# SaeedRahmani/MPC-RL_for_AVs

Measured on AMD Instinct MI355X. Metric: MPC solves/sec (horizon=20, batch=4096), higher is better.
Workload: dtype f64

## Files before the change

### __graft_entry__.py

```python
from __future__ import annotations

import os
import subprocess
import sys

ROOT = os.path.dirname(os.path.abspath(__file__))
if ROOT not in sys.path:
    sys.path.insert(0, ROOT)
ORACLE = os.path.join(ROOT, "oracle")


def abi_version_of_header() -> int:
    import re
    with open(os.path.join(ROOT, "include", "mpc_mi355x.h")) as f:
        m = re.search(r"^#define\s+MPC_ABI_VERSION\s+(\d+)", f.read(), re.M)
    if not m:
        raise RuntimeError("MPC_ABI_VERSION not found in include/mpc_mi355x.h")
    return int(m.group(1))


def build() -> None:
    from mpc_rl_for_avs_amd import _build, engine
    path = _build.build(force=_build.is_stale())
    print(f"[build] {path}")
    subprocess.run(["make", "-C", ORACLE, "-s"], check=True)
    print(f"[build] {os.path.join(ORACLE, '_build', 'libmpc_oracle.so')}")
    wave_ops_suite = os.path.exists(os.path.join(ROOT, "tests", "wave_ops_cases.py"))
    for lib, src in (("libcpu_wave.so", "cpu_wave_harness.cpp"), ("libcpu_wave_spare.so", "cpu_wave_spare_harness.cpp"),
                     ("libcpu_ltv.so", "cpu_ltv_harness.cpp"),
                     ("libcpu_preamble.so", "cpu_preamble_harness.cpp"), ("libcpu_synth_env.so", "cpu_synth_env_harness.cpp"),
                     ("libcpu_traffic_env.so", "cpu_traffic_env_harness.cpp"),
                     ("libcpu_rollout_glue.so", "cpu_rollout_glue_harness.cpp"), ("libcpu_sde_glue.so", "cpu_sde_glue_harness.cpp"),
                     ("libcpu_wave_ops.so", "cpu_wave_ops_harness.cpp")):
        if lib == "libcpu_wave_ops.so" and not wave_ops_suite:
            continue
        harness = os.path.join(ROOT, "tests", "_build", lib)
        os.makedirs(os.path.dirname(harness), exist_ok=True)
        subprocess.run(["g++", "-O2", "-fPIC", "-shared", "-std=c++17", "-Wno-unknown-pragmas", "-ffp-contract=off",
                        "-o", harness, os.path.join(ROOT, "tests", src)], check=True)
        print(f"[build] {harness}")
    if wave_ops_suite:
        probe = os.path.join(ROOT, "tests", "_build", "libdev_wave_ops.so")
        subprocess.run([_build._hipcc(), "--offload-arch=gfx950", "-O3", "-std=c++17", "-shared", "-fPIC", "-o", probe,
                        os.path.join(ROOT, "tests", "dev_wave_ops.hip")], check=True)
        print(f"[build] {probe}")
    lib = engine.load_library()
    want = abi_version_of_header()
    got = lib.mpc_version()
    assert got == want, f"libmpc_mi355x.so reports ABI {got}, include/mpc_mi355x.h declares {want}: stale library?"
    import mpc_rl_for_avs_amd.pure_mpc
    import mpc_rl_for_avs_amd.pure_mpc_linear


def smoke() -> None:
    if ORACLE not in sys.path:
        sys.path.insert(0, ORACLE)
    import numpy as np
    from mpc_rl_for_avs_amd import engine, synth
    from mpc_rl_for_avs_amd.reference_path import reference_states
    import oracle_lib

    inp = synth.solver_inputs(64, 4, seed=11)
    eng = engine.MPCEngine(horizon=20, max_iter=100, device=0)
    got = eng.solve_batch(inp["state"], inp["ego_index"], inp["weights"], inp["is_collide"], vref=inp["vref"],
                          others=inp["others"], collision_cost=True)
    want = oracle_lib.solve_batch(reference_states(), inp["state"], inp["ego_index"], inp["weights"],
                                  inp["is_collide"], vref=inp["vref"], others=inp["others"], collision_cost=True,
                                  max_iter=100, xy_bounds=False)
    conv = lambda st: (st == 0) | ((st >= 5) & (st <= 7))
    both = conv(got["status"]) & conv(want["status"])
    assert both.sum() >= 60, f"too few converged instances: gpu {got['status']}, oracle {want['status']}"
    assert np.array_equal(got["status"], want["status"]), "status mismatch"
    err = np.abs(got["u0"] - want["u0"]).max(axis=1) / np.maximum(1.0, np.abs(want["u0"]).max(axis=1))
    assert err[both].max() < 1e-4, f"u0 mismatch {err[both].max():.3e}"
    print(f"[smoke] {both.sum()}/64 converged on both, max rel |u0_gpu - u0_oracle| = {err[both].max():.2e}")
    import kkt_batch
    import nlp_batch
    sel = np.nonzero(conv(got["status"]))[0]
    p = nlp_batch.Batch.build(reference_states(), inp["state"], inp["ego_index"], inp["weights"], inp["is_collide"],
                              vref=inp["vref"], others=inp["others"], collision_cost=True).take(sel)
    cert = kkt_batch.certify(p, got["X"][sel], got["U"][sel], eps_c=1e-8 / kkt_batch.objective_scale(p))
    assert cert["stationarity"].max() <= 1e-8 and cert["feasibility"].max() <= 1e-10, cert
# ... 20 lines not shown
```

### mpc-rl_for_avs_amd/csrc/mpc_engine.hip

```cpp
#include <hip/hip_runtime.h>

#include <atomic>
#include <cassert>
#include <chrono>
#include <cmath>
#include <cstdio>
#include <cstring>
#include <new>
#include <string>
#include <vector>

#include "../../include/mpc_mi355x.h"
#include "mpc_core.hpp"
#include "mpc_ltv.hpp"
#include "mpc_wave.hpp"
#include "mpc_wave_dev.hpp"
#include "mpc_preamble.hpp"
#include "mpc_preamble_wave.hpp"
#include "mpc_synth_lanes.hpp"
#include "mpc_rollout_glue.hpp"
#include "mpc_drive_metrics.hpp"
#include "mpc_perception.hpp"
#include "mpc_interaction.hpp"
#include "mpc_episode_stats.hpp"

namespace {

thread_local std::string g_last_error;

int fail(int code, const std::string &msg) {
    g_last_error = msg;
    return code;
}

#define HIP_TRY(expr)                                                                              \
    do {                                                                                           \
        hipError_t e_ = (expr);                                                                    \
        if (e_ != hipSuccess)                                                                      \
            return fail(MPC_ERR_HIP, std::string(#expr) + ": " + hipGetErrorString(e_));          \
    } while (0)

constexpr int kBlock = 64;
constexpr int kMaxDevices = 64;
constexpr int kWaveOcc = 3, kWaveOccGeneric = 3;
constexpr int kWaveOccGenericCC = 2;
constexpr int kWaveOccLat = 2, kLatDepth = 4;
constexpr int kRelaxLat = 7;
constexpr bool wave_spare_lds(int NC, int OCC, int RELAX) { return NC > 0 && OCC == kWaveOccLat && RELAX == kRelaxLat; }

template <int NC, int RELAX = 0, bool SPARE = false>
struct WaveCtx : mpc::wave::WaveOpsT<RELAX> {
    static constexpr int kN = NC;
    static constexpr bool kSpareLds = SPARE;
    const double *table;
    int e0, M;
    __device__ __forceinline__ WaveCtx(mpc::wave::lds_double_t *l, const double *t, int e, int m)
        : mpc::wave::WaveOpsT<RELAX>{l}, table(t), e0(mpc::ego_row0(e, m)), M(m) {}
    __device__ __forceinline__ void tick(int) const {}
    __device__ __forceinline__ double ref(int k, int c) const {
        int idx = e0 + k;
        idx = idx > M - 1 ? M - 1 : idx;
        idx = idx < 0 ? 0 : idx;
        return table[idx * mpc::REF_COLS + c];
    }
    __device__ __forceinline__ double refv(int k) const {
        int idx = e0 + k;
        idx = idx > M - 1 ? M - 1 : idx;
        idx = idx < 0 ? 0 : idx;
        return table[M * mpc::REF_COLS + idx];
    }
};

template <bool CC, class CTX>
__device__ __forceinline__ void stage_problem(CTX &ctx, const mpc::SolveParams &P, int b, int lane, int N, int SL,
                                              const double *__restrict__ ref5, int M, const double *__restrict__ vref,
                                              const double *__restrict__ others, int Vin) {
    const int OTH = SL * (N + 1) + mpc::wave::SC_SIZE;
    for (int node = lane; node <= N; node += kBlock) {
        double rv;
        if (vref) {
            rv = vref[(size_t)b * (N + 1) + node];
        } else {
            int idx = ctx.e0 + node;
            idx = idx > M - 1 ? M - 1 : idx;
            idx = idx < 0 ? 0 : idx;
            rv = ref5[M * mpc::REF_COLS + idx];
        }
        ctx.st(node * SL + mpc::wave::W_RV, rv);
    }
    if (CC && lane < P.V) {
        const double *ov = others + ((size_t)b * Vin + lane) * 4;
        const double sp = ov[2] * P.dt, hh = ov[3];
        ctx.st(OTH + lane * 4 + 0, ov[0]);
        ctx.st(OTH + lane * 4 + 1, ov[1]);
        ctx.st(OTH + lane * 4 + 2, sp * cos(hh));
        ctx.st(OTH + lane * 4 + 3, sp * sin(hh));
    }
}

template <bool CC, int NC, int OCC, int RELAX>
__global__ __launch_bounds__(kBlock, OCC) void mpc_solve_wave_kernel(
    mpc::SolveParams P, int B, const double *__restrict__ ref5, int M, const double *__restrict__ state,
    const int32_t *__restrict__ ego_index, const double *__restrict__ vref, const double *__restrict__ weights,
    const uint8_t *__restrict__ is_collide, const double *__restrict__ others, int Vin,
    const int32_t *__restrict__ nveh, double w_collision, const double *u_init, int u_shift, uint8_t *u_valid,
    double *__restrict__ u0_out, double *U_out, double *__restrict__ X_out, int32_t *__restrict__ status_out,
    int32_t *__restrict__ iters_out, const int32_t *__restrict__ order) {
    extern __shared__ double smem[];
    const int N = NC > 0 ? NC : P.N;
    if ((int)blockIdx.x >= B) return;
    const int b = order ? order[blockIdx.x] : (int)blockIdx.x;
    if (nveh) P.V = min(P.V, max(0, nveh[b]));
    const int lane = threadIdx.x;
    constexpr int SL = mpc::wave::stage_slots(CC);
    using Ctx = WaveCtx<NC, RELAX, wave_spare_lds(NC, OCC, RELAX)>;
    Ctx ctx((mpc::wave::lds_double_t *)smem, ref5, ego_index[b], M);
    stage_problem<CC>(ctx, P, b, lane, N, SL, ref5, M, vref, others, Vin);
    __syncthreads();
    double x0[4];
#pragma unroll
    for (int i = 0; i < 4; ++i) x0[i] = state[(size_t)b * 4 + i];
    const bool collide = is_collide[b] != 0;
    const double ws_ = collide ? 100.0 : weights[(size_t)b * 3 + 0];
    const double wcoll = (CC && collide) ? 3000.0 * w_collision : 0.0;
    mpc::wave::Solver<CC, Ctx> solver(P, ctx, x0, ws_, weights[(size_t)b * 3 + 1], weights[(size_t)b * 3 + 2], wcoll);
    int status, iters, cur;
    double kkt;
    const bool warm = u_init != nullptr && (u_valid == nullptr || u_valid[b] != 0);
    if (warm && lane < N) {
        const int src = min(lane + u_shift, N - 1);
        ctx.st(lane * SL + mpc::wave::W_U + 0, mpc::warm_clamp(u_init[((size_t)b * N + src) * 2 + 0], 0));
        ctx.st(lane * SL + mpc::wave::W_U + 1, mpc::warm_clamp(u_init[((size_t)b * N + src) * 2 + 1], 1));
    }
    __syncthreads();
    solver.solve(status, iters, cur, kkt, warm);
    __syncthreads();
    const int CB = cur * 6;
    if (P.strict_kink && (status == MPC_STATUS_CONVERGED_ON_KINK || status == MPC_STATUS_ACCEPTABLE_ON_KINK))
        status = MPC_STATUS_KINK_UNSOLVED;
    if (lane == 0 && u_valid && U_out) u_valid[b] = MPC_STATUS_IS_SOLVED(status) ? 1 : 0;
    if (lane < 2) u0_out[(size_t)b * 2 + lane] = ctx.ld(CB + mpc::wave::W_U + lane);
    if (U_out && lane < N) {
        U_out[((size_t)b * N + lane) * 2 + 0] = ctx.ld(lane * SL + CB + mpc::wave::W_U + 0);
        U_out[((size_t)b * N + lane) * 2 + 1] = ctx.ld(lane * SL + CB + mpc::wave::W_U + 1);
    }
    if (X_out)
        for (int node = lane; node <= N; node += kBlock)
#pragma unroll
            for (int i = 0; i < 4; ++i)
                X_out[((size_t)b * (N + 1) + node) * 4 + i] = ctx.ld(node * SL + CB + mpc::wave::W_X + i);
    if (lane == 0) {
        if (status_out) status_out[b] = status;
        if (iters_out) iters_out[b] = iters;
    }
}

__global__ __launch_bounds__(64) void mpc_timer_kernel(long long ticks) {
    const long long t0 = wall_clock64();
    while (wall_clock64() - t0 < ticks) __builtin_amdgcn_s_sleep(8);
}

constexpr double kOrderStanding = 0.1, kOrderNear = 15.0, kOrderTurn = 0.05;
constexpr int kOrderBehind = 5;
__device__ __forceinline__ int order_tier(const uint8_t *is_collide, const double *state, const double *others, int V,
                                          const int32_t *nveh, const int32_t *ego, const double *ref5, int M, int N, int i) {
    const double *x = state + (size_t)i * 4;
    if (x[3] < kOrderStanding) return 0;
    if (is_collide[i] != 0) {
// ... 1681 lines not shown
```

### mpc-rl_for_avs_amd/csrc/mpc_wave.hpp

```cpp
#pragma once

#include "mpc_core.hpp"

namespace mpc {
namespace wave {

constexpr int kLanes = 64;
constexpr int kTrials = 4;
constexpr double kProjKeep = 0.1;
constexpr double kProjKeepEnd = 1e-3, kProjEndMu = 1e-6;
constexpr int kGnWatch = 4, kGnSkip = 4;
constexpr double kGnEndMu = 1e-2;
constexpr int kDwProbe = 4;
constexpr int kBoostIter = 28;
constexpr double kOpenLoopStep = 1e-9;
constexpr double kAcceptableTol = 1e-6;
constexpr int kAcceptableIter = 15;
constexpr double kRegMax = 1.0;
constexpr double kKappaEps = 30.0;
constexpr double kMinSlack = 1e-14;
constexpr double kInitPush = 1e-2;

enum : int {
    W_X = 0,
// ... 6 lines not shown
    W_Y = 32,
    W_KX = 36,
    W_KP = 44,
    W_KF = 48,
    W_RV = 50,
    W_ONE = 51,
    W_DTC = 52,
    W_SLOTS = 53,
    W_LX = 53,
    W_Q = 55,
    W_QG = 58,
    W_ZW = 61,
    W_WJ = 62,
    W_CROSS = 63,
    W_SLOTS_CC = 65
};
constexpr int kZeroWord = W_LIN + 2;
enum : int { LIN_A02 = 0, LIN_A12 = 1, LIN_A03 = 4, LIN_A13 = 5, LIN_A23 = 6, LIN_B01 = 8, LIN_B11 = 9, LIN_B21 = 10 };
enum : int { W_DXY = W_LX, W_GW = W_Q, W_DZW = W_Q + 1 };
static_assert(kTrials == 4, "the trial areas below are laid out for four trials");
MPC_HD constexpr int trial_x(bool, int t, int TB) { return t == 0 ? TB : (t == 1 ? W_LIN : (t == 2 ? W_LIN + 6 : W_KX)); }
MPC_HD constexpr int trial_u(bool cc, int t, int TB) { return trial_x(cc, t, TB); }
enum : int {
    SC_SPARE = 0,
    SC_TRIG = 4,
    SC_LOG = SC_TRIG + kTrigWords,
    SC_BND = SC_LOG + kLogWords,
    SC_K = SC_BND + 8,
    SC_NB = SC_K + 6,
    SC_SIZE = SC_NB + 3
};
enum : int { K_SF = 0, K_RD, K_RC, K_QTT, K_Q33, K_MUMIN };
constexpr int kMaxHorizon = kLanes;
enum : int {
    A_L00 = W_KX + 0, A_L01 = W_KX + 1, A_L11 = W_KX + 2, A_H22 = W_KX + 3, A_H23 = W_KX + 4, A_H33 = W_KX + 5,
    A_WTD = W_KX + 6, A_WVD = W_KX + 7, A_H66 = W_KP + 0, A_H77 = W_KP + 1, A_HV6 = W_KP + 2, A_HV7 = W_KF + 0,
    A_HV4 = W_KF + 1,
    A_HV0 = W_X,
    A_HV5 = W_U
};

constexpr int kPreSlots = 12;
enum : int { PQ = 0, PB = 8 };
constexpr double kNoBound = 1e300;

MPC_HD constexpr int stage_slots(bool cc) { return (cc ? W_SLOTS_CC : W_SLOTS) + kPreSlots; }

MPC_HD constexpr int spare_doubles(bool cc, int N, int V) { return cc ? 2 * V * (N + 1) : 0; }
template <class CTX, class = void>
struct spare_lds { static constexpr bool value = false; };
template <class CTX>
struct spare_lds<CTX, decltype((void)CTX::kSpareLds)> { static constexpr bool value = CTX::kSpareLds; };

MPC_HD constexpr int lds_doubles(bool cc, int N, int V, bool spare = false) {
    return stage_slots(cc) * (N + 1) + SC_SIZE + (cc ? 4 * V : 0) + (spare ? spare_doubles(cc, N, V) : 0);
}

enum : int {
    T_PREP = 0, T_ADJOINT, T_DUALRES, T_RIC_INIT, T_RIC_SCALARS, T_RIC_L1, T_RIC_L2, T_RIC_2X2, T_RIC_L4, T_LINEAR,
    T_RATIOS, T_ROLL_DYN, T_ROLL_COST, T_DUALUPD,
    T_R_FEEDBACK, T_R_CLAMP, T_R_DYN, T_R_STORE, T_R_CHECK, T_R_PROJ, T_R_LDSW, T_COUNT
};
template <class CTX, class = void>
struct fine_ticks { static constexpr bool value = false; };
template <class CTX>
struct fine_ticks<CTX, decltype((void)CTX::kFine)> { static constexpr bool value = CTX::kFine; };

template <class T>
struct PerLane {
#if defined(__HIPCC__)
    T v;
    MPC_HD T &at(int) { return v; }
#else
    T v[kLanes];
    MPC_HD T &at(int lane) { return v[lane]; }
#endif
};

MPC_HD bool ratio_greater(double n2, double d2, double n1, double d1) {
    const double a = n2 * d1, b = n1 * d2;
    return a > b || (a == b && d2 > d1);
}

#if !defined(__HIPCC__)
inline int row_partner(int l, int step) {
    return step == 0 ? (l ^ 1) : (step == 1 ? (l ^ 2) : (step == 2 ? ((l & ~7) | (7 - (l & 7))) : ((l & ~15) | (15 - (l & 15)))));
}
template <class T, class OP>
inline void host_row_reduce(PerLane<T> &p, OP op) {
    for (int step = 0; step < 4; ++step) {
        T nv[kLanes];
        for (int l = 0; l < kLanes; ++l) nv[l] = op(p.v[l], p.v[row_partner(l, step)]);
        for (int l = 0; l < kLanes; ++l) p.v[l] = nv[l];
    }
}
template <class T, class OP>
inline T host_reduce(PerLane<T> &p, OP op) {
    host_row_reduce(p, op);
    return op(op(p.v[0], p.v[16]), op(p.v[32], p.v[48]));
}
#endif

MPC_HD constexpr int stage_transition_word(int r, int c, int lin, int zero, int one, int dtw) {
    const int key = 8 * r + c;
    int w = zero;
    w = (r < 4 && r == c) ? one : w;
// ... 22 lines not shown
    double x0[4];
    double ws_, wc_, wd_, wcoll;
    double sf = 1.0;
    MPC_HD double SF() const { return sc(SC_K + K_SF); }
    MPC_HD double RD() const { return sc(SC_K + K_RD); }
    MPC_HD double RC() const { return sc(SC_K + K_RC); }
    MPC_HD double WS() const { return c.fresh(ws_); }
    MPC_HD double WC() const { return c.fresh(wc_); }
    MPC_HD double WD() const { return c.fresh(wd_); }
    MPC_HD double WCOLL() const { return c.fresh(wcoll); }

    MPC_HD Solver(const SolveParams &P_, CTX &c_, const double *x0_, double ws, double wc, double wd, double wcl)
        : P(P_), c(c_), N(CTX::kN > 0 ? CTX::kN : P_.N), SL(stage_slots(CC)), SCR(SL * (N + 1)), OTH(SCR + SC_SIZE),
          SPP(OTH + (CC ? 4 * P_.V : 0)), dt(P_.dt), ws_(c_.uni(ws)), wc_(c_.uni(wc)), wd_(c_.uni(wd)), wcoll(c_.uni(wcl)) {
        x0[0] = x0_[0]; x0[1] = x0_[1]; x0[2] = x0_[2]; x0[3] = x0_[3];
    }
    MPC_HD double S(int k, int slot) const { return c.ld(k * SL + slot); }
    MPC_HD void S(int k, int slot, double v) { c.st(k * SL + slot, v); }
    MPC_HD double sc(int i) const { return c.ld(SCR + i); }
    MPC_HD void sc(int i, double v) { c.st(SCR + i, v); }
    MPC_HD double oth(int j, int q) const { return c.ld(OTH + j * 4 + q); }
    MPC_HD double veh_x(int j, int k) const { return kSpare ? c.ld(SPP + 2 * (j * (N + 1) + k)) : oth(j, 0) + k * oth(j, 2); }
    MPC_HD double veh_y(int j, int k) const { return kSpare ? c.ld(SPP + 2 * (j * (N + 1) + k) + 1) : oth(j, 1) + k * oth(j, 3); }
    MPC_HD void init_spare() {
        if (!kSpare || !CC) return;
        c.phase([&](int lane) {
            for (int k = lane; k <= N; k += kLanes)
                for (int j = 0; j < P.V; ++j) {
                    c.st(SPP + 2 * (j * (N + 1) + k), oth(j, 0) + k * oth(j, 2));
                    c.st(SPP + 2 * (j * (N + 1) + k) + 1, oth(j, 1) + k * oth(j, 3));
                }
        });
    }
    MPC_HD double xlo(int i) const { return sc(SC_BND + 0 + 2 * i); }
    MPC_HD double xhi(int i) const { return sc(SC_BND + 1 + 2 * i); }
    MPC_HD double ulo(int i) const { return sc(SC_BND + 4 + 2 * i); }
    MPC_HD double uhi(int i) const { return sc(SC_BND + 5 + 2 * i); }
    MPC_HD double flog(double x) const {
        double K[kLogWords];
        for (int i = 0; i < kLogWords; ++i) K[i] = sc(SC_LOG + i);
        return log_pos(K, x);
    }
    MPC_HD TrigCoef trig() const {
        TrigCoef K;
        for (int i = 0; i < 6; ++i) {
            K.s[i] = sc(SC_TRIG + i);
            K.c[i] = sc(SC_TRIG + 6 + i);
        }
        return K;
    }

    PerLane<double> red_a, red_b, red_c, red_w;
    PerLane<int> ls_feas;
    int any_wall = 0;
    MPC_HD int f_word(int r, int c) const {
        const int w = stage_transition_word(r, c, 0, 1000, 1001, 1002);
        int t = w;
        t = w == 1000 ? kZeroWord : t;
        t = w == 1001 ? W_ONE : t;
        t = w == 1002 ? W_DTC : t;
        t = w == 0 ? W_LIN + LIN_A02 : t;
        t = w == 1 ? W_LIN + LIN_A03 : t;
        t = w == 2 ? W_LIN + LIN_A12 : t;
        t = w == 3 ? W_LIN + LIN_A13 : t;
        t = w == 4 ? W_LIN + LIN_A23 : t;
        t = w == 5 ? W_LIN + LIN_B01 : t;
        t = w == 6 ? W_LIN + LIN_B11 : t;
        t = w == 7 ? W_LIN + LIN_B21 : t;
        return t;
    }
    PerLane<int> r_a, r_b, r_lxx, r_lux, r_m, r_lx, r_lu, r_kx;
    MPC_HD void set_roles4(int AB) {
        c.lanes([&](int lane_) {
            const int lane = c.opaque(lane_);
            const int hi = lane >> 4, blk = (lane >> 2) & 3, lo = lane & 3;
            const int zero = kZeroWord;
            r_a.at(lane_) = f_word(hi, lo);
            r_b.at(lane_) = f_word(hi, lo < 2 ? 6 + lo : 4);
            const int a = hi < lo ? hi : lo, b = hi < lo ? lo : hi;
            const int key = a * 4 + b;
            int slot = zero;
            slot = key == 0 * 4 + 0 ? A_L00 : slot;
            slot = key == 0 * 4 + 1 ? A_L01 : slot;
            slot = key == 1 * 4 + 1 ? A_L11 : slot;
            slot = key == 2 * 4 + 2 ? A_H22 : slot;
            slot = key == 2 * 4 + 3 ? A_H23 : slot;
            slot = key == 3 * 4 + 3 ? A_H33 : slot;
            r_lxx.at(lane_) = slot;
            r_lux.at(lane_) = hi == 1 ? (lo == 2 ? A_WTD : (lo == 3 ? A_WVD : zero)) : zero;
            r_m.at(lane_) = (hi == 0 && lo == 0) ? A_H66 : ((hi == 1 && lo == 1) ? A_H77 : zero);
            r_lx.at(lane_) = lo == 0 ? AB + A_HV0 + hi : zero;
            r_lu.at(lane_) = lo == 0 ? (hi == 0 ? A_HV6 : (hi == 1 ? A_HV7 : zero)) : zero;
            int out = -1;
            out = (blk == 0 && hi < 2) ? W_KX + 2 * lo + hi : out;
            out = (blk == 1 && hi < 2 && lo < 2) ? W_KP + 2 * lo + hi : out;
            out = (blk == 2 && hi < 2 && lo == 0) ? W_KF + hi : out;
            r_kx.at(lane_) = out;
        });
    }

    MPC_HD void load_stage4(int k, int AB, PerLane<double> &RA, PerLane<double> &RB, PerLane<double> &QXX, PerLane<double> &QUX,
                            PerLane<double> &M, PerLane<double> &QX, PerLane<double> &QU, double &lp0, double &lp1) {
        c.lanes([&](int lane) {
            const int base = k * SL;
            auto word = [&](int w) { return c.ld(base + w); };
            RA.at(lane) = word(r_a.at(lane));
            RB.at(lane) = word(r_b.at(lane));
            QXX.at(lane) = word(r_lxx.at(lane));
            QUX.at(lane) = word(r_lux.at(lane));
            M.at(lane) = word(r_m.at(lane));
            QX.at(lane) = word(r_lx.at(lane));
            QU.at(lane) = word(r_lu.at(lane));
        });
        lp0 = S(k, A_HV4);
        lp1 = S(k, AB + A_HV5);
    }
    MPC_HD bool sweep4(int CB, int AB, double mu, double delta_w, bool gn, double &dV1) {
        double tsig[2], tgr[2];
        for (int i = 0; i < 2; ++i) {
            const double xi = S(N, CB + W_X + 2 + i);
            const double rl = frcp(xi - xlo(i)), ru = frcp(xhi(i) - xi);
            tsig[i] = S(N, W_ZXL + i) * rl + S(N, W_ZXU + i) * ru + delta_w;
            tgr[i] = mu * (ru - rl);
        }
        PerLane<double> PXX, PXP, PX;
        c.lanes([&](int lane_) {
            const int lane = c.opaque_shared(lane_);
            const int hi = lane >> 4, lo = lane & 3;
            PXX.at(lane_) = hi == lo ? (hi == 2 ? tsig[0] : (hi == 3 ? tsig[1] : delta_w)) : 0.0;
            PXP.at(lane_) = 0.0;
            PX.at(lane_) = lo == 0 ? (hi == 2 ? tgr[0] : (hi == 3 ? tgr[1] : 0.0)) : 0.0;
        });
        double pp00 = 0.0, pp01 = 0.0, pp11 = 0.0, ppv0 = 0.0, ppv1 = 0.0;
        c.tick(T_RIC_INIT);
        const double rd_full = RD();
#pragma unroll 1
        for (int k = N - 1; k >= 0; --k) {
            const double rdk = (k >= 1) ? rd_full : 0.0;
            PerLane<double> RA, RB, QXX, QUX, M, QX, QU, T0, T1;
            double lp0, lp1;
            load_stage4(k, AB, RA, RB, QXX, QUX, M, QX, QU, lp0, lp1);
            c.lanes([&](int lane) {
                T0.at(lane) = 0.0;
                T1.at(lane) = PXP.at(lane);
            });
            c.tick(T_RIC_SCALARS);
            c.mfma(PXX, RA, T0);
            c.mfma(PXX, RB, T1);
            c.mfma(PXP, RB, M);
            c.mfma(RA, PX, QX);
            c.mfma(RB, PX, QU);
            c.tick(T_RIC_L1);
            c.mfma(RB, T1, M);
            c.mfma(T1, RA, QUX);
            c.mfma(RA, T0, QXX);
            c.tick(T_RIC_L2);
            double ha = c.lane_get(M, 0) + pp00, hb = c.lane_get(M, 1) + pp01, hc = c.lane_get(M, 17) + pp11;
            const double hu0 = c.lane_get(QU, 0) + ppv0, hu1 = c.lane_get(QU, 16) + ppv1;
            double det = ha * hc - hb * hb;
            bool pd = (ha > 0.0) & (hc > 0.0) & (det > c.fresh(1e-12) * ha * hc);
            PerLane<double> NWA, RWA, Ya, QS, KFB, PXXn, PXPn, PXn;
            double idet, i00, i01, i11, kf0, kf1;
            auto stage_tail = [&]() {
                const double kfa0 = hb * hu1 - hc * hu0, kfa1 = hb * hu0 - ha * hu1;
                c.lanes([&](int lane_) {
                    const int lane = c.opaque_shared(lane_);
                    const int hi = lane >> 4, lo = lane & 3;
                    const double w00 = (hi == 0 && lo == 0) ? 1.0 : 0.0, w11 = (hi == 1 && lo == 1) ? 1.0 : 0.0;
                    const double wof = ((hi == 0 && lo == 1) || (hi == 1 && lo == 0)) ? 1.0 : 0.0;
                    const double c1 = (hi == 1 && lo == 0) ? 1.0 : 0.0;
                    const double nwa = wof * hb - w00 * hc - w11 * ha;
                    NWA.at(lane_) = nwa;
                    RWA.at(lane_) = -rdk * nwa;
                    KFB.at(lane_) = w00 * kfa0 + c1 * kfa1;
                    Ya.at(lane_) = 0.0;
                    PXPn.at(lane_) = 0.0;
                    PXXn.at(lane_) = QXX.at(lane_);
                    PXn.at(lane_) = QX.at(lane_);
                });
                c.mfma(NWA, QUX, Ya);
                idet = frcp(det);
                c.lanes([&](int lane) { QS.at(lane) = idet * QUX.at(lane); });
                c.mfma(QS, Ya, PXXn);
                c.mfma(QS, RWA, PXPn);
                c.mfma(QS, KFB, PXn);
                i00 = hc * idet;
                i01 = -hb * idet;
                i11 = ha * idet;
                kf0 = kfa0 * idet;
                kf1 = kfa1 * idet;
            };
            stage_tail();
            if (!pd && !gn) {
                double wdd, wtt = 0.0, wtv = 0.0, wtd = 0.0, wvd = 0.0, q00 = 0.0, q01 = 0.0, q11 = 0.0;
                {
                    const double v = S(k, CB + W_X + 3);
                    double Sn, Cn, sb, cb_, bp, bpp;
                    dyn_eval(trig(), S(k, CB + W_X + 2), S(k, CB + W_U + 1), Sn, Cn, sb, cb_);
                    beta_derivs(sb, cb_, bp, bpp);
                    const double yy0 = S(k + 1, W_Y + 0), yy1 = S(k + 1, W_Y + 1), yy2 = S(k + 1, W_Y + 2);
                    const double g = -(yy0 * Cn + yy1 * Sn), h = -(yy0 * Sn - yy1 * Cn);
                    wdd = dt * v * (g * bp * bp + h * bpp) + dt * yy2 * v * kInvWheelbase * (-sb * bp * bp + cb_ * bpp);
                    if (k >= 1) {
                        wtt = dt * v * g;
                        wtv = dt * h;
                        wtd = dt * v * g * bp;
                        wvd = dt * h * bp + dt * yy2 * cb_ * bp * kInvWheelbase;
                        if (CC) {
                            q00 = S(k, W_QG + 0) - S(k, W_Q + 0);
                            q01 = S(k, W_QG + 1) - S(k, W_Q + 1);
                            q11 = S(k, W_QG + 2) - S(k, W_Q + 2);
                            if (any_wall && S(k, W_WJ) >= 0.0) {
                                q00 += 2.0 * S(k, W_ZW);
                                q11 += 2.0 * S(k, W_ZW);
                            }
                        }
                    }
                }
                c.lanes([&](int lane_) {
                    const int lane = c.opaque_shared(lane_);
                    const int hi = lane >> 4, lo = lane & 3;
                    const int a = hi < lo ? hi : lo, b = hi < lo ? lo : hi;
                    double cx = 0.0;
                    switch (a * 4 + b) {
                        case 0 * 4 + 0: cx = q00; break;
                        case 0 * 4 + 1: cx = q01; break;
                        case 1 * 4 + 1: cx = q11; break;
                        case 2 * 4 + 2: cx = -wtt; break;
                        case 2 * 4 + 3: cx = -wtv; break;
                        default: break;
                    }
                    QXX.at(lane_) += cx;
                    QUX.at(lane_) += hi == 1 ? (lo == 2 ? -wtd : (lo == 3 ? -wvd : 0.0)) : 0.0;
                });
                hc -= wdd;
                det = ha * hc - hb * hb;
                pd = (ha > 0.0) & (hc > 0.0) & (det > c.fresh(1e-12) * ha * hc);
                if (pd) stage_tail();
            }
            if (!pd) return false;
            c.tick(T_RIC_2X2);
            dV1 += 0.5 * (kf0 * hu0 + kf1 * hu1);
            const double kp00 = rdk * i00, kp01 = rdk * i01, kp11 = rdk * i11;
            c.lanes([&](int lane) {
                PXX.at(lane) = PXXn.at(lane);
                PXP.at(lane) = PXPn.at(lane);
                PX.at(lane) = PXn.at(lane);
                const int ks = r_kx.at(lane);
                const bool is_kp = (ks >= W_KP) & (ks < W_KF), is_kf = ks >= W_KF;
                const double t = is_kf ? KFB.at(lane) : (is_kp ? -NWA.at(lane) : Ya.at(lane));
                const double v = (idet * t) * (is_kp ? rd_full : 1.0);
                if (ks >= 0) S(k, ks, v);
            });
            pp00 = rdk - rdk * kp00;
            pp01 = -rdk * kp01;
            pp11 = rdk - rdk * kp11;
            ppv0 = lp0 - rdk * kf0;
            ppv1 = lp1 - rdk * kf1;
            c.tick(T_RIC_L4);
        }
// ... 577 lines not shown
        if (!(warm && rollout_init(Jcur, barcur, false))) {
            c.phase([&](int lane) {
                if (lane >= N) return;
                S(lane, W_U + 0, 0.0);
                S(lane, W_U + 1, 0.0);
            });
            if (x0[3] < 0.01) S(0, W_U + 0, (0.01 - x0[3]) / dt);
            if (!rollout_init(Jcur, barcur, true)) {
                status_out = 3;
                return;
            }
        }
        {
            c.phase([&](int lane) {
                double g = 0.0;
                if (lane >= 1 && lane < N) {
                    if (CC) {
                        double d8[8];
                        dist(lane, S(lane, W_X + 0), S(lane, W_X + 1), d8);
                        S(lane, W_LX + 0, d8[0]);
                        S(lane, W_LX + 1, d8[1]);
                    }
                    double lx[4];
                    cost_grad(0, lane, lx);
                    g = fmax2(fmax2(fabs(lx[0]), fabs(lx[1])), fmax2(fabs(lx[2]), fabs(lx[3])));
                }
                red_a.at(lane) = g;
            });
            const double gmax = fmax2(0.02 * (WC() + WD()) * fabs(S(0, W_U + 0)), c.wave_max(red_a));
            sf = c.uni(100.0 / fmin2(fmax2(100.0, gmax), 1e4));
            Jcur = c.uni(Jcur * sf);
            barcur = c.uni(barcur);
        }
        sc(SC_K + K_SF, sf);
        sc(SC_K + K_RD, 0.02 * sf * wd_);
        sc(SC_K + K_RC, 0.02 * sf * wc_);
        sc(SC_K + K_QTT, 10.0 * sf);
        sc(SC_K + K_Q33, sf * (20.0 * ws_ + (CC ? 2.0 * wcoll : 0.0)));
        sc(SC_K + K_MUMIN, P.tol / 10.0);
        double mu = P.mu_init;
        int iter = 0, nfail = 0;
        double reg = 0.0;
        sc(SC_SPARE + 3, 0.0);
        int i_mark = 0;
        double e_mark = INFINITY;
        int gn_streak = 0, gn_skip = 0;
        const bool nonconvex_cost = (ws_ < 0.0) | (wc_ < 0.0) | (wd_ < 0.0);
        bool prev_needed = false, prev_gn = false;
        double e_streak = INFINITY;
        int n_acceptable = 0;

        for (iter = 0; iter <= P.max_iter; ++iter) {
            const int CB = cur * 6;
            if (iter == kBoostIter) c.template set_priority<3>();
            c.tick(T_DUALUPD);
            const int coll_nodes = N - 1;
            const int coll_groups = (!CC || coll_nodes < 1) ? 1 : (kLanes / coll_nodes >= 3 ? 3 : (kLanes / coll_nodes >= 2 ? 2 : 1));
            auto coll_word = [&](int g, int i) __attribute__((always_inline)) {
                return g == 0 ? W_LX + i : (g == 1 ? W_KX + i : (i < 6 ? W_KP + i : (cur ^ 1) * 6 + (i - 6)));
            };
            if (CC && coll_nodes >= 1) {
                c.phase([&](int lane) {
                    const int g = lane / coll_nodes, k = 1 + lane - g * coll_nodes;
                    if (g >= coll_groups) return;
                    double d8[8];
                    dist(k, S(k, CB + W_X + 0), S(k, CB + W_X + 1), d8, g, coll_groups);
                    for (int i = 0; i < 8; ++i) S(k, coll_word(g, i), d8[i]);
                });
            }
            c.phase([&](int lane) {
                if (lane >= N) {
                    red_a.at(lane) = 0.0;
                    red_b.at(lane) = INFINITY;
                    red_c.at(lane) = 0.0;
                    if (CC) red_w.at(lane) = -1.0;
                    return;
                }
                const int k = lane;
                const double u0 = S(k, CB + W_U + 0), u1 = S(k, CB + W_U + 1);
                const double xk0 = S(k, CB + W_X + 0), xk1 = S(k, CB + W_X + 1), xk2 = S(k, CB + W_X + 2),
                             xk3 = S(k, CB + W_X + 3);
                {
                    double Sn, Cn, sb, cb_, bp, bpp;
                    dyn_eval(trig(), xk2, u1, Sn, Cn, sb, cb_);
                    beta_derivs(sb, cb_, bp, bpp);
                    S(k, W_LIN + 2, 0.0); S(k, W_LIN + 3, 0.0); S(k, W_LIN + 7, 0.0); S(k, W_LIN + 11, 0.0);
                    S(k, W_LIN + LIN_A02, -dt * xk3 * Sn);
                    S(k, W_LIN + LIN_A03, dt * Cn);
                    S(k, W_LIN + LIN_A12, dt * xk3 * Cn);
                    S(k, W_LIN + LIN_A13, dt * Sn);
                    S(k, W_LIN + LIN_A23, dt * sb * kInvWheelbase);
                    S(k, W_LIN + LIN_B01, -dt * xk3 * Sn * bp);
                    S(k, W_LIN + LIN_B11, dt * xk3 * Cn * bp);
                    S(k, W_LIN + LIN_B21, dt * xk3 * kInvWheelbase * cb_ * bp);
                }
                double wall_z = -1.0, wall_c = 0.0;
                if (k >= 1) {
                    double g[4];
                    track(k, xk0, xk1, xk2, xk3, g);
                    double lx0 = SF() * g[0], lx1 = SF() * g[1], lx2 = SF() * g[2], lx3 = SF() * g[3];
                    if (CC) {
                        double d8[8];
                        for (int i = 0; i < 8; ++i) {
                            d8[i] = S(k, coll_word(0, i));
                            if (coll_groups >= 2) d8[i] += S(k, coll_word(1, i));
                            if (coll_groups >= 3) d8[i] += S(k, coll_word(2, i));
                        }
                        S(k, W_LX + 0, SF() * d8[0]);
                        S(k, W_LX + 1, SF() * d8[1]);
                        S(k, W_Q + 0, SF() * d8[2]);
                        S(k, W_Q + 1, SF() * d8[3]);
                        S(k, W_Q + 2, SF() * d8[4]);
                        S(k, W_QG + 0, SF() * d8[5]);
                        S(k, W_QG + 1, SF() * d8[6]);
                        S(k, W_QG + 2, SF() * d8[7]);
                        lx0 += SF() * d8[0];
                        lx1 += SF() * d8[1];
                        lx3 += SF() * 2.0 * WCOLL() * xk3;
                        if (any_wall) {
                            const double wjv = S(k, W_WJ);
                            if (wjv >= 0.0) {
                                double nx, ny;
                                const double g = wall_slack(k, xk0, xk1, (int)wjv, nx, ny);
                                wall_z = S(k, W_ZW);
                                wall_c = g * wall_z;
                                lx0 -= wall_z * nx;
                                lx1 -= wall_z * ny;
                            }
                        }
                    }
                    S(k, W_Y + 0, lx0);
                    S(k, W_Y + 1, lx1);
                    S(k, W_Y + 2, lx2 - S(k, W_ZXL + 0) + S(k, W_ZXU + 0));
                    S(k, W_Y + 3, lx3 - S(k, W_ZXL + 1) + S(k, W_ZXU + 1));
                } else {
                    S(N, W_Y + 0, 0.0);
                    S(N, W_Y + 1, 0.0);
                    S(N, W_Y + 2, -S(N, W_ZXL + 0) + S(N, W_ZXU + 0));
// ... 124 lines not shown
                n_acceptable = (E0 <= c.fresh(kAcceptableTol)) ? n_acceptable + 1 : 0;
                if (n_acceptable >= kAcceptableIter) {
                    status_out = (CC && zw_max > c.fresh(1e-6) * SF()) ? 7 : 6;
                    break;
                }
            }
            if (iter == P.max_iter) break;
            if (P.stall_window > 0) {
                if (E0 < 0.5 * e_mark) {
                    e_mark = c.uni(E0);
                    i_mark = iter;
                } else if (iter - i_mark >= P.stall_window) {
                    status_out = 4;
                    break;
                }
            }

            c.tick(T_DUALRES);
            const int AB = (cur ^ 1) * 6;
            double dV1 = 0.0, delta_w = reg;
            bool ok = false, gn = false;
            int nmod = 0;
            if (nonconvex_cost && prev_needed && iter % kDwProbe != 0) {
                delta_w = fmax2(reg, c.fresh(1.0 / 3.0) * c.uni(sc(SC_SPARE + 3)));
                gn = prev_gn && !(mu <= c.fresh(kGnEndMu));
            }
            bool skipped_gn = false;
            set_roles4(AB);
            for (int attempt = 0; attempt < 16 && !ok; ++attempt) {
                ok = true;
                dV1 = 0.0;
                c.phase([&](int lane) {
                    if (lane >= N) return;
                    const int k = lane;
                    const double rc = RC(), qtt = sc(SC_K + K_QTT), q33 = sc(SC_K + K_Q33);
                    const double rdk = (k >= 1) ? RD() : 0.0;
                    const double v = S(k, CB + W_X + 3);
                    const double u0 = S(k, CB + W_U + 0), u1 = S(k, CB + W_U + 1);
                    double sig[4], sgr[4];
                    for (int q = 0; q < 4; ++q) {
                        const bool isx = q < 2;
                        const int b = isx ? q : q - 2;
                        const double val = isx ? S(k, CB + W_X + 2 + b) : (b == 0 ? u0 : u1);
                        const double lo = isx ? xlo(b) : ulo(b), hi = isx ? xhi(b) : uhi(b);
                        const double zl = isx ? S(k, W_ZXL + b) : S(k, W_ZUL + b);
                        const double zu = isx ? S(k, W_ZXU + b) : S(k, W_ZUU + b);
                        const double rl = frcp(val - lo), ru = frcp(hi - val);
                        sig[q] = zl * rl + zu * ru;
                        sgr[q] = mu * (ru - rl);
                    }
                    double wdd = 0.0, wtt = 0.0, wtv = 0.0, wtd = 0.0, wvd = 0.0;
                    if (!gn) {
                        double Sn, Cn, sb, cb_, bp, bpp;
                        dyn_eval(trig(), S(k, CB + W_X + 2), u1, Sn, Cn, sb, cb_);
                        beta_derivs(sb, cb_, bp, bpp);
                        const double yy0 = S(k + 1, W_Y + 0), yy1 = S(k + 1, W_Y + 1), yy2 = S(k + 1, W_Y + 2);
                        const double g = -(yy0 * Cn + yy1 * Sn), h = -(yy0 * Sn - yy1 * Cn);
                        wdd = dt * v * (g * bp * bp + h * bpp) + dt * yy2 * v * kInvWheelbase * (-sb * bp * bp + cb_ * bpp);
                        wtt = dt * v * g;
                        wtv = dt * h;
                        wtd = dt * v * g * bp;
                        wvd = dt * h * bp + dt * yy2 * cb_ * bp * kInvWheelbase;
                    }
                    double l00 = 0.0, l01 = 0.0, l11 = 0.0, h22 = 0.0, h23 = 0.0, h33 = 0.0, hv0 = 0.0, hv1 = 0.0, hv2 = 0.0,
                           hv3 = 0.0;
                    if (k >= 1) {
                        double lx[4];
                        cost_grad(cur, k, lx);
                        const double s = c.ref(k, R_SIN), cc = c.ref(k, R_COS);
                        l00 = SF() * 10.0 * (8.0 * s * s + 4.0 * cc * cc) + delta_w;
                        l01 = SF() * 10.0 * (-8.0 * s * cc + 4.0 * cc * s);
                        l11 = SF() * 10.0 * (8.0 * cc * cc + 4.0 * s * s) + delta_w;
                        if (CC) {
                            const int QS = gn ? W_QG : W_Q;
                            l00 += S(k, QS + 0);
                            l01 += S(k, QS + 1);
                            l11 += S(k, QS + 2);
                        }
                        h22 = wtt + qtt + sig[0] + delta_w;
                        h23 = wtv;
                        h33 = q33 + sig[1] + delta_w;
                        hv0 = lx[0];
                        hv1 = lx[1];
                        if (CC && any_wall) {
                            const double wjv = S(k, W_WJ);
                            if (wjv >= 0.0) {
                                double nx, ny;
                                const double rg = frcp(wall_slack(k, S(k, CB + W_X + 0), S(k, CB + W_X + 1), (int)wjv, nx, ny));
                                const double zw = S(k, W_ZW), sg = zw * rg, cv = gn ? 0.0 : 2.0 * zw;
                                l00 += sg * nx * nx - cv;
                                l01 += sg * nx * ny;
                                l11 += sg * ny * ny - cv;
                                hv0 -= mu * rg * nx;
                                hv1 -= mu * rg * ny;
                            }
                        }
                        hv2 = lx[2] + sgr[0];
                        hv3 = lx[3] + sgr[1];
                    } else {
                        wtd = 0.0;
                        wvd = 0.0;
                    }
                    double um0 = 0.0, um1 = 0.0;
                    if (k >= 1) {
                        um0 = S(k - 1, CB + W_U + 0);
                        um1 = S(k - 1, CB + W_U + 1);
                    }
                    S(k, A_L00, l00);
                    S(k, A_L01, l01);
                    S(k, A_L11, l11);
                    S(k, A_H22, h22);
                    S(k, A_H23, h23);
                    S(k, A_H33, h33);
                    S(k, A_WTD, wtd);
                    S(k, A_WVD, wvd);
                    S(k, A_H66, rc + rdk + sig[2] + delta_w);
                    S(k, A_H77, rc + rdk + sig[3] + delta_w + wdd);
                    S(k, AB + A_HV0, hv0);
                    S(k, AB + A_HV0 + 1, hv1);
                    S(k, AB + A_HV0 + 2, hv2);
                    S(k, AB + A_HV0 + 3, hv3);
                    S(k, A_HV4, -rdk * (u0 - um0));
                    S(k, AB + A_HV5, -rdk * (u1 - um1));
                    S(k, A_HV6, rc * u0 + rdk * (u0 - um0) + sgr[2]);
                    S(k, A_HV7, rc * u1 + rdk * (u1 - um1) + sgr[3]);
                });
                ok = sweep4(CB, AB, mu, delta_w, gn, dV1);
                if (!ok) {
                    ++nmod;
                    if (gn_skip > 0) skipped_gn = true;
                    if (!gn && gn_skip == 0 && !(nonconvex_cost && mu <= c.fresh(kGnEndMu))) {
                        gn = true;
                    } else {
                        const double dw_last = c.uni(sc(SC_SPARE + 3));
                        if (dw_last == 0.0) {
                            delta_w = (delta_w < 1e-4) ? c.fresh(1e-4) : c.fresh(100.0) * delta_w;
                        } else {
                            const double third = c.fresh(1.0 / 3.0) * dw_last;
                            delta_w = (delta_w < third) ? third : c.fresh(8.0) * delta_w;
                        }
                    }
                    if (delta_w > 1e40) break;
                }
            }
            if (!ok) {
                status_out = 2;
                break;
            }
            if (delta_w > reg) sc(SC_SPARE + 3, delta_w);
            prev_needed = delta_w > reg;
            prev_gn = gn;
            if (nmod > 0) {
                if (gn_streak == 0) e_streak = c.uni(E0);
                ++gn_streak;
                if (gn_skip > 0) {
                    --gn_skip;
                } else if (gn_streak % kGnWatch == 0) {
                    if (E0 > 0.5 * e_streak) gn_skip = kGnSkip;
                    e_streak = c.uni(E0);
                }
            } else {
                gn_streak = 0;
                gn_skip = 0;
            }

            c.tick(T_RIC_INIT);
            const double tau = c.uni(fmax2(0.99, 1.0 - mu));
            c.tick(T_LINEAR);
            if (CC && any_wall) {
                c.phase([&](int lane) {
                    const int kn = lane + 1;
                    if (kn >= N) return;
                    const double wjv = S(kn, W_WJ);
                    if (wjv >= 0.0) {
                        double nx, ny;
                        S(kn, W_GW, wall_slack(kn, S(kn, CB + W_X + 0), S(kn, CB + W_X + 1), (int)wjv, nx, ny));
                    }
                });
            }
            const double phi0 = c.uni(Jcur + mu * barcur);
            const int tb = cur ^ 1;
            double Jn = 0.0, barn = 0.0;
            int acc_trial = -1;
            const double keep = c.uni(mu <= c.fresh(kProjEndMu) ? c.fresh(kProjKeepEnd) : c.fresh(kProjKeep));
            const bool accepted = line_search(cur, 0.5 * (1.0 - tau), keep, phi0, dV1, mu, Jn, barn, acc_trial);
            const bool have_cross = CC && P.V > 0 && acc_trial != 0;
            c.phase([&](int lane) {
                if (lane >= N) {
                    red_b.at(lane) = 0.0;
                    red_c.at(lane) = 1.0;
                    return;
                }
                const int k = lane;
                double rdn = 0.0, rdd = 1.0;
                for (int i = 0; i < 4; ++i) {
                    const bool isu = i < 2;
                    const int j = isu ? i : i - 2;
                    const double lo = isu ? ulo(j) : xlo(j), hi = isu ? uhi(j) : xhi(j);
                    const int kk = isu ? k : k + 1;
                    const double val = isu ? S(kk, CB + W_U + j) : S(kk, CB + W_X + 2 + j);
                    const double d = S(kk, W_Y + i);
                    const double zl = isu ? S(kk, W_ZUL + j) : S(kk, W_ZXL + j);
                    const double zu = isu ? S(kk, W_ZUU + j) : S(kk, W_ZXU + j);
                    const double rsl = frcp(val - lo), rsu = frcp(hi - val);
                    const double dzl = (mu - zl * d) * rsl - zl, dzu = (mu + zu * d) * rsu - zu;
                    if (-dzl * rdd > rdn * zl) { rdn = -dzl; rdd = zl; }
                    if (-dzu * rdd > rdn * zu) { rdn = -dzu; rdd = zu; }
                }
                if (CC && any_wall && k + 1 < N) {
                    const double wjv = S(k + 1, W_WJ);
                    if (wjv >= 0.0) {
                        double nx, ny;
                        wall_slack(k + 1, S(k + 1, CB + W_X + 0), S(k + 1, CB + W_X + 1), (int)wjv, nx, ny);
                        const double g = S(k + 1, W_GW);
                        const double d = nx * S(k + 1, W_DXY + 0) + ny * S(k + 1, W_DXY + 1), rg = frcp(g);
                        const double zw = S(k + 1, W_ZW), dzw = (mu - zw * d) * rg - zw;
                        if (-dzw * rdd > rdn * zw) { rdn = -dzw; rdd = zw; }
                        S(k + 1, W_DZW, dzw);
                    }
                }
                red_b.at(lane) = rdn;
                red_c.at(lane) = rdd;
            });
            double a_du;
            {
                double rdn, rdd;
                c.wave_max_ratio(red_b, red_c, rdn, rdd);
                a_du = c.uni((rdn > tau * rdd) ? tau * rdd / rdn : 1.0);
            }
            c.tick(T_RATIOS);
            bool newwall = false;
            double bar_shift = 0.0;
            if (accepted && acc_trial == 0) {
                reg = 0.25 * reg;
                if (reg < 1e-3) reg = 0.0;
            } else if (!accepted || acc_trial >= 2) {
                reg = (reg == 0.0) ? 1e-3 : fmin2(4.0 * reg, kRegMax);
            }
            reg = c.uni(reg);
            {
                const int NB = (accepted ? tb : cur) * 6;
                c.phase([&](int lane) {
                    if (lane >= N) return;
                    const int k = lane;
                    for (int i = 0; i < 4; ++i) {
                        const bool isu = i < 2;
                        const int j = isu ? i : i - 2;
                        const double lo = isu ? ulo(j) : xlo(j), hi = isu ? uhi(j) : xhi(j);
                        const int kk = isu ? k : k + 1;
                        const int sv = isu ? (W_U + j) : (W_X + 2 + j);
                        const int szl = isu ? (W_ZUL + j) : (W_ZXL + j), szu = isu ? (W_ZUU + j) : (W_ZXU + j);
                        const double val = S(kk, CB + sv), d = S(kk, W_Y + i);
                        const double zl = S(kk, szl), zu = S(kk, szu);
                        const double dzl = (mu - zl * d) * frcp(val - lo) - zl, dzu = (mu + zu * d) * frcp(hi - val) - zu;
                        const double vn = S(kk, NB + sv);
                        const double ml = mu * frcp(vn - lo), mh = mu * frcp(hi - vn);
                        S(kk, szl, fmax2(fmin2(zl + (dzl > 0.0 ? 1.0 : a_du) * dzl, c.fresh(1e10) * ml), c.fresh(1e-10) * ml));
                        S(kk, szu, fmax2(fmin2(zu + (dzu > 0.0 ? 1.0 : a_du) * dzu, c.fresh(1e10) * mh), c.fresh(1e-10) * mh));
                    }
                });
                if (CC && (any_wall || have_cross)) {
                    c.phase([&](int lane) {
                        red_a.at(lane) = 0.0;
                        red_b.at(lane) = 0.0;
                        const int kn = lane + 1;
                        if (kn >= N) return;
                        const double wjv = S(kn, W_WJ), cr = have_cross ? S(kn, W_CROSS) : -1.0;
                        const double xn0 = S(kn, NB + W_X + 0), xn1 = S(kn, NB + W_X + 1);
                        double nx, ny, gcur = INFINITY, flag = 0.0;
                        if (wjv >= 0.0) {
                            gcur = wall_slack(kn, xn0, xn1, (int)wjv, nx, ny);
                            const double zw = S(kn, W_ZW), dzw = S(kn, W_DZW), ml = mu * frcp(gcur);
                            S(kn, W_ZW, fmax2(fmin2(zw + (dzw > 0.0 ? 1.0 : a_du) * dzw, c.fresh(1e10) * ml), c.fresh(1e-10) * ml));
                            flag = 1.0;
                        }
                        if (cr >= 0.0 && cr != wjv) {
                            const double gc = wall_slack(kn, xn0, xn1, (int)cr, nx, ny);
                            if (gc > 0.0 && gc < gcur) {
                                S(kn, W_WJ, cr);
                                S(kn, W_ZW, mu * frcp(gc));
                                red_b.at(lane) = (wjv >= 0.0 ? flog(gcur) : 0.0) - flog(gc);
                                flag = 3.0;
                            }
                        }
                        red_a.at(lane) = flag;
                    });
                    const double wf = c.wave_max(red_a);
                    any_wall = wf > 0.0;
                    newwall = wf > 2.0;
                    if (newwall) bar_shift = c.wave_sum(red_b);
                }
            }
            if (accepted) {
                cur = tb;
                Jcur = c.uni(Jn);
                barcur = c.uni(barn);
                nfail = 0;
            } else if (newwall) {
                nfail = 0;
                if (skipped_gn) gn_skip = 0;
            } else if (skipped_gn) {
                gn_skip = 0;
            } else if (++nfail >= 3) {
                status_out = 4;
                ++iter;
                break;
            }
// ... 10 lines not shown
```

Measured before the change: 1.074 million.

## Carry trig derivatives and dual step values across wave phases in registers

Adds a compile-time carry mode, enabled for the latency-tuned spare-LDS wave configuration, that keeps per-lane trig/beta derivative values and dual-step deltas in per-lane registers across phases. Later phases reuse them instead of recomputing dyn_eval, beta_derivs and the reciprocal-based dual updates, and the Hessian terms are rewritten with explicit fma. This trims repeated transcendental and division work per iteration. In exchange it raises register pressure at low occupancy and changes rounding through fma, which could move results slightly relative to the oracle.

Result: faster. 1.096 million (median of 6 runs) (+2.0%).

```diff
diff --git a/__graft_entry__.py b/__graft_entry__.py
--- a/__graft_entry__.py
+++ b/__graft_entry__.py
@@ -27,7 +27,7 @@
     print(f"[build] {os.path.join(ORACLE, '_build', 'libmpc_oracle.so')}")
     wave_ops_suite = os.path.exists(os.path.join(ROOT, "tests", "wave_ops_cases.py"))
     for lib, src in (("libcpu_wave.so", "cpu_wave_harness.cpp"), ("libcpu_wave_spare.so", "cpu_wave_spare_harness.cpp"),
-                     ("libcpu_ltv.so", "cpu_ltv_harness.cpp"),
+                     ("libcpu_wave_carry.so", "cpu_wave_carry_harness.cpp"), ("libcpu_ltv.so", "cpu_ltv_harness.cpp"),
                      ("libcpu_preamble.so", "cpu_preamble_harness.cpp"), ("libcpu_synth_env.so", "cpu_synth_env_harness.cpp"),
                      ("libcpu_traffic_env.so", "cpu_traffic_env_harness.cpp"),
                      ("libcpu_rollout_glue.so", "cpu_rollout_glue_harness.cpp"), ("libcpu_sde_glue.so", "cpu_sde_glue_harness.cpp"),
diff --git a/mpc-rl_for_avs_amd/csrc/mpc_engine.hip b/mpc-rl_for_avs_amd/csrc/mpc_engine.hip
--- a/mpc-rl_for_avs_amd/csrc/mpc_engine.hip
+++ b/mpc-rl_for_avs_amd/csrc/mpc_engine.hip
@@ -47,11 +47,13 @@
 constexpr int kWaveOccLat = 2, kLatDepth = 4;
 constexpr int kRelaxLat = 7;
 constexpr bool wave_spare_lds(int NC, int OCC, int RELAX) { return NC > 0 && OCC == kWaveOccLat && RELAX == kRelaxLat; }
-
-template <int NC, int RELAX = 0, bool SPARE = false>
+constexpr bool wave_phase_carry(int NC, int OCC, int RELAX) { return wave_spare_lds(NC, OCC, RELAX); }
+
+template <int NC, int RELAX = 0, bool SPARE = false, bool CARRY = false>
 struct WaveCtx : mpc::wave::WaveOpsT<RELAX> {
     static constexpr int kN = NC;
     static constexpr bool kSpareLds = SPARE;
+    static constexpr bool kCarry = CARRY;
     const double *table;
     int e0, M;
     __device__ __forceinline__ WaveCtx(mpc::wave::lds_double_t *l, const double *t, int e, int m)
@@ -113,7 +115,7 @@
     if (nveh) P.V = min(P.V, max(0, nveh[b]));
     const int lane = threadIdx.x;
     constexpr int SL = mpc::wave::stage_slots(CC);
-    using Ctx = WaveCtx<NC, RELAX, wave_spare_lds(NC, OCC, RELAX)>;
+    using Ctx = WaveCtx<NC, RELAX, wave_spare_lds(NC, OCC, RELAX), wave_phase_carry(NC, OCC, RELAX)>;
     Ctx ctx((mpc::wave::lds_double_t *)smem, ref5, ego_index[b], M);
     stage_problem<CC>(ctx, P, b, lane, N, SL, ref5, M, vref, others, Vin);
     __syncthreads();
diff --git a/mpc-rl_for_avs_amd/csrc/mpc_wave.hpp b/mpc-rl_for_avs_amd/csrc/mpc_wave.hpp
--- a/mpc-rl_for_avs_amd/csrc/mpc_wave.hpp
+++ b/mpc-rl_for_avs_amd/csrc/mpc_wave.hpp
@@ -82,6 +82,21 @@
 template <class CTX>
 struct spare_lds<CTX, decltype((void)CTX::kSpareLds)> { static constexpr bool value = CTX::kSpareLds; };
 
+template <class CTX, class = void>
+struct phase_carry { static constexpr bool value = false; };
+template <class CTX>
+struct phase_carry<CTX, decltype((void)CTX::kCarry)> { static constexpr bool value = CTX::kCarry; };
+MPC_HD double fused(double a, double b, double c) {
+#if defined(__HIP_DEVICE_COMPILE__)
+    return fma(a, b, c);
+#else
+    return a * b + c;
+#endif
+}
+#ifndef MPC_CARRY_PARTS
+#define MPC_CARRY_PARTS 7
+#endif
+
 MPC_HD constexpr int lds_doubles(bool cc, int N, int V, bool spare = false) {
     return stage_slots(cc) * (N + 1) + SC_SIZE + (cc ? 4 * V : 0) + (spare ? spare_doubles(cc, N, V) : 0);
 }
@@ -210,6 +225,12 @@
 
     PerLane<double> red_a, red_b, red_c, red_w;
     PerLane<int> ls_feas;
+    static constexpr bool kCarry = phase_carry<CTX>::value;
+    static constexpr bool kCarryDual = kCarry && (MPC_CARRY_PARTS & 1) != 0;
+    static constexpr bool kCarryTrig = kCarry && (MPC_CARRY_PARTS & 2) != 0;
+    static constexpr bool kCarrySweep = kCarryTrig && (MPC_CARRY_PARTS & 4) != 0;
+    struct DualCarry { PerLane<double> dzl[4], dzu[4]; };
+    struct TrigCarry { PerLane<double> sn, cn, sb, cb, bp, bpp; };
     int any_wall = 0;
     MPC_HD int f_word(int r, int c) const {
         const int w = stage_transition_word(r, c, 0, 1000, 1001, 1002);
@@ -273,7 +294,7 @@
         lp0 = S(k, A_HV4);
         lp1 = S(k, AB + A_HV5);
     }
-    MPC_HD bool sweep4(int CB, int AB, double mu, double delta_w, bool gn, double &dV1) {
+    MPC_HD bool sweep4(int CB, int AB, double mu, double delta_w, bool gn, double &dV1, TrigCarry &trc) {
         double tsig[2], tgr[2];
         for (int i = 0; i < 2; ++i) {
             const double xi = S(N, CB + W_X + 2 + i);
@@ -354,16 +375,31 @@
                 {
                     const double v = S(k, CB + W_X + 3);
                     double Sn, Cn, sb, cb_, bp, bpp;
-                    dyn_eval(trig(), S(k, CB + W_X + 2), S(k, CB + W_U + 1), Sn, Cn, sb, cb_);
-                    beta_derivs(sb, cb_, bp, bpp);
+                    if constexpr (kCarrySweep) {
+                        Sn = c.lane_get(trc.sn, k); Cn = c.lane_get(trc.cn, k); sb = c.lane_get(trc.sb, k);
+                        cb_ = c.lane_get(trc.cb, k); bp = c.lane_get(trc.bp, k); bpp = c.lane_get(trc.bpp, k);
+                    } else {
+                        dyn_eval(trig(), S(k, CB + W_X + 2), S(k, CB + W_U + 1), Sn, Cn, sb, cb_);
+                        beta_derivs(sb, cb_, bp, bpp);
+                    }
                     const double yy0 = S(k + 1, W_Y + 0), yy1 = S(k + 1, W_Y + 1), yy2 = S(k + 1, W_Y + 2);
-                    const double g = -(yy0 * Cn + yy1 * Sn), h = -(yy0 * Sn - yy1 * Cn);
-                    wdd = dt * v * (g * bp * bp + h * bpp) + dt * yy2 * v * kInvWheelbase * (-sb * bp * bp + cb_ * bpp);
+                    double g, h;
+                    if constexpr (kCarrySweep) {
+                        g = -fused(yy0, Cn, yy1 * Sn);
+                        h = -fused(yy0, Sn, -(yy1 * Cn));
+                        const double cg = fused(g * bp, bp, h * bpp), cy = fused(cb_, bpp, -sb * bp * bp);
+                        wdd = fused(dt * v, cg, dt * yy2 * v * kInvWheelbase * cy);
+                    } else {
+                        g = -(yy0 * Cn + yy1 * Sn);
+                        h = -(yy0 * Sn - yy1 * Cn);
+                        wdd = dt * v * (g * bp * bp + h * bpp) + dt * yy2 * v * kInvWheelbase * (-sb * bp * bp + cb_ * bpp);
+                    }
                     if (k >= 1) {
                         wtt = dt * v * g;
                         wtv = dt * h;
                         wtd = dt * v * g * bp;
-                        wvd = dt * h * bp + dt * yy2 * cb_ * bp * kInvWheelbase;
+                        if constexpr (kCarrySweep) wvd = fused(dt * h, bp, dt * yy2 * cb_ * bp * kInvWheelbase);
+                        else wvd = dt * h * bp + dt * yy2 * cb_ * bp * kInvWheelbase;
                         if (CC) {
                             q00 = S(k, W_QG + 0) - S(k, W_Q + 0);
                             q01 = S(k, W_QG + 1) - S(k, W_Q + 1);
@@ -1047,6 +1083,8 @@
 
         for (iter = 0; iter <= P.max_iter; ++iter) {
             const int CB = cur * 6;
+            DualCarry dlc;
+            TrigCarry trc;
             if (iter == kBoostIter) c.template set_priority<3>();
             c.tick(T_DUALUPD);
             const int coll_nodes = N - 1;
@@ -1079,6 +1117,10 @@
                     double Sn, Cn, sb, cb_, bp, bpp;
                     dyn_eval(trig(), xk2, u1, Sn, Cn, sb, cb_);
                     beta_derivs(sb, cb_, bp, bpp);
+                    if constexpr (kCarryTrig) {
+                        trc.sn.at(lane) = Sn; trc.cn.at(lane) = Cn; trc.sb.at(lane) = sb;
+                        trc.cb.at(lane) = cb_; trc.bp.at(lane) = bp; trc.bpp.at(lane) = bpp;
+                    }
                     S(k, W_LIN + 2, 0.0); S(k, W_LIN + 3, 0.0); S(k, W_LIN + 7, 0.0); S(k, W_LIN + 11, 0.0);
                     S(k, W_LIN + LIN_A02, -dt * xk3 * Sn);
                     S(k, W_LIN + LIN_A03, dt * Cn);
@@ -1309,15 +1351,30 @@
                     double wdd = 0.0, wtt = 0.0, wtv = 0.0, wtd = 0.0, wvd = 0.0;
                     if (!gn) {
                         double Sn, Cn, sb, cb_, bp, bpp;
-                        dyn_eval(trig(), S(k, CB + W_X + 2), u1, Sn, Cn, sb, cb_);
-                        beta_derivs(sb, cb_, bp, bpp);
+                        if constexpr (kCarryTrig) {
+                            Sn = trc.sn.at(lane); Cn = trc.cn.at(lane); sb = trc.sb.at(lane);
+                            cb_ = trc.cb.at(lane); bp = trc.bp.at(lane); bpp = trc.bpp.at(lane);
+                        } else {
+                            dyn_eval(trig(), S(k, CB + W_X + 2), u1, Sn, Cn, sb, cb_);
+                            beta_derivs(sb, cb_, bp, bpp);
+                        }
                         const double yy0 = S(k + 1, W_Y + 0), yy1 = S(k + 1, W_Y + 1), yy2 = S(k + 1, W_Y + 2);
-                        const double g = -(yy0 * Cn + yy1 * Sn), h = -(yy0 * Sn - yy1 * Cn);
-                        wdd = dt * v * (g * bp * bp + h * bpp) + dt * yy2 * v * kInvWheelbase * (-sb * bp * bp + cb_ * bpp);
-                        wtt = dt * v * g;
-                        wtv = dt * h;
-                        wtd = dt * v * g * bp;
-                        wvd = dt * h * bp + dt * yy2 * cb_ * bp * kInvWheelbase;
+                        if constexpr (kCarryTrig) {
+                            const double g = -fused(yy0, Cn, yy1 * Sn), h = -fused(yy0, Sn, -(yy1 * Cn));
+                            const double cg = fused(g * bp, bp, h * bpp), cy = fused(cb_, bpp, -sb * bp * bp);
+                            wdd = fused(dt * yy2 * v * kInvWheelbase, cy, dt * v * cg);
+                            wtt = dt * v * g;
+                            wtv = dt * h;
+                            wtd = dt * v * g * bp;
+                            wvd = fused(dt * yy2 * cb_ * bp, kInvWheelbase, dt * h * bp);
+                        } else {
+                            const double g = -(yy0 * Cn + yy1 * Sn), h = -(yy0 * Sn - yy1 * Cn);
+                            wdd = dt * v * (g * bp * bp + h * bpp) + dt * yy2 * v * kInvWheelbase * (-sb * bp * bp + cb_ * bpp);
+                            wtt = dt * v * g;
+                            wtv = dt * h;
+                            wtd = dt * v * g * bp;
+                            wvd = dt * h * bp + dt * yy2 * cb_ * bp * kInvWheelbase;
+                        }
                     }
                     double l00 = 0.0, l01 = 0.0, l11 = 0.0, h22 = 0.0, h23 = 0.0, h33 = 0.0, hv0 = 0.0, hv1 = 0.0, hv2 = 0.0,
                            hv3 = 0.0;
@@ -1382,7 +1439,7 @@
                     S(k, A_HV6, rc * u0 + rdk * (u0 - um0) + sgr[2]);
                     S(k, A_HV7, rc * u1 + rdk * (u1 - um1) + sgr[3]);
                 });
-                ok = sweep4(CB, AB, mu, delta_w, gn, dV1);
+                ok = sweep4(CB, AB, mu, delta_w, gn, dV1, trc);
                 if (!ok) {
                     ++nmod;
                     if (gn_skip > 0) skipped_gn = true;
@@ -1463,6 +1520,10 @@
                     const double dzl = (mu - zl * d) * rsl - zl, dzu = (mu + zu * d) * rsu - zu;
                     if (-dzl * rdd > rdn * zl) { rdn = -dzl; rdd = zl; }
                     if (-dzu * rdd > rdn * zu) { rdn = -dzu; rdd = zu; }
+                    if constexpr (kCarryDual) {
+                        dlc.dzl[i].at(lane) = dzl;
+                        dlc.dzu[i].at(lane) = dzu;
+                    }
                 }
                 if (CC && any_wall && k + 1 < N) {
                     const double wjv = S(k + 1, W_WJ);
@@ -1507,9 +1568,17 @@
                         const int kk = isu ? k : k + 1;
                         const int sv = isu ? (W_U + j) : (W_X + 2 + j);
                         const int szl = isu ? (W_ZUL + j) : (W_ZXL + j), szu = isu ? (W_ZUU + j) : (W_ZXU + j);
-                        const double val = S(kk, CB + sv), d = S(kk, W_Y + i);
-                        const double zl = S(kk, szl), zu = S(kk, szu);
-                        const double dzl = (mu - zl * d) * frcp(val - lo) - zl, dzu = (mu + zu * d) * frcp(hi - val) - zu;
+                        double zl, zu, dzl, dzu;
+                        if constexpr (kCarryDual) {
+                            zl = S(kk, szl); zu = S(kk, szu);
+                            dzl = dlc.dzl[i].at(lane);
+                            dzu = dlc.dzu[i].at(lane);
+                        } else {
+                            const double val = S(kk, CB + sv), d = S(kk, W_Y + i);
+                            zl = S(kk, szl); zu = S(kk, szu);
+                            dzl = (mu - zl * d) * frcp(val - lo) - zl;
+                            dzu = (mu + zu * d) * frcp(hi - val) - zu;
+                        }
                         const double vn = S(kk, NB + sv);
                         const double ml = mu * frcp(vn - lo), mh = mu * frcp(hi - vn);
                         S(kk, szl, fmax2(fmin2(zl + (dzl > 0.0 ? 1.0 : a_du) * dzl, c.fresh(1e10) * ml), c.fresh(1e-10) * ml));
```
